# alexoz12v2/cuda-optix-pathtracing

Hardware: AMD Instinct MI355X
Metric: Msamples/s (paths x spp / s) (higher is better)
Workload: dtype f32

## Files before the change

### cuda-optix-pathtracing_amd/__init__.py

```python
from .binding import (
    DmtError,
    Renderer,
    bvh_validate,
    bvh_check,
    lbvh_reference,
    BVH_BUILD_HOST,
    BVH_BUILD_DEVICE,
    BVH_BUILT_BY_HOST,
    BVH_BUILT_BY_DEVICE,
    BVH_BUILT_BY_HOST_AFTER_DEVICE,
    bvh_refit_reference,
    BVH_UPDATE_REBUILD,
    BVH_UPDATE_REFIT,
    BVH_UPDATE_AUTO,
    BVH_UPDATED_NONE,
    BVH_UPDATED_REFIT,
    BVH_UPDATED_REBUILD,
    BVH_UPDATED_REBUILD_AFTER_REFIT,
    light_tree_pmfs,
    light_tree_ref_select,
    envmap_tables,
    texture_mip_chain,
    texture_footprint,
    temporal_defaults,
    camera_project,
    lens_rays,
    shutter_times,
    motion_positions,
    motion_bvh_validate,
    smooth_normals,
    opacity_eval,
    OPACITY_NONE,
    medium_segment,
    medium_values,
    phase_hg,
    medium_grid_march,
    medium_spectrum_event,
    mip_level_count,
    TEXFILTER_LEVEL0,
    TEXFILTER_REFERENCE,
    build_library,
    library_path,
    load_library,
)
from . import host_scene
from . import multigpu
```

### cuda-optix-pathtracing_amd/binding.py

```python
import ctypes as C
import subprocess
from pathlib import Path

import numpy as np

_HERE = Path(__file__).resolve().parent
_CSRC = _HERE / "csrc"
_LIB = None

DMT_ACCEL_BRUTE_FORCE = 0
DMT_ACCEL_BVH = 1
BVH_BUILD_HOST = 0
BVH_BUILD_DEVICE = 1
BVH_BUILT_BY_HOST = 0
BVH_BUILT_BY_DEVICE = 1
BVH_BUILT_BY_HOST_AFTER_DEVICE = 2
BVH_UPDATE_REBUILD = 0
BVH_UPDATE_REFIT = 1
BVH_UPDATE_AUTO = 2
BVH_UPDATED_NONE = 0
BVH_UPDATED_REFIT = 1
BVH_UPDATED_REBUILD = 2
BVH_UPDATED_REBUILD_AFTER_REFIT = 3

# ... 20 lines not shown
    global _LIB
    if _LIB is None:
        so = library_path()
        if not so.exists():
            raise DmtError(f"{so} is missing: run `python -c 'import __graft_entry__ as g; g.build()'` "
                           "(the HIP path has no fallback)")
        lib = C.CDLL(str(so))
        lib.dmt_last_error.restype = C.c_char_p
        lib.dmt_last_error.argtypes = [C.c_void_p]
        _LIB = lib
    return _LIB


EXPORTED_SYMBOLS = [
    "dmt_ctx_create", "dmt_ctx_destroy", "dmt_last_error", "dmt_upload_triangles", "dmt_upload_bsdfs",
    "dmt_upload_lights", "dmt_set_camera", "dmt_set_limits", "dmt_set_accel", "dmt_set_light_sampling", "dmt_light_tree_pmfs", "dmt_light_tree_ref_select", "dmt_set_bvh_strategy", "dmt_set_partition", "dmt_set_chunk", "dmt_render_profile",
    "dmt_upload_area_lights", "dmt_upload_textures", "dmt_upload_envmap", "dmt_clear_envmap", "dmt_envmap_tables", "dmt_test_envmap",
    "dmt_set_stream", "dmt_film_clear", "dmt_film_bind", "dmt_film_device_ptrs", "dmt_download_film",
    "dmt_render", "dmt_render_adaptive", "dmt_render_stats", "dmt_sync", "dmt_sched_diag", "dmt_kernel_time", "dmt_kernel_info", "dmt_bvh_validate", "dmt_brute_cull_plan", "dmt_brute_cull_box_plan", "dmt_brute_cull_box_records", "dmt_cull_box_test", "dmt_test_triangle_intersect",
    "dmt_test_sampler", "dmt_test_camera_rays", "dmt_test_bsdf", "dmt_test_bsdf_ng", "dmt_test_material", "dmt_test_light", "dmt_test_half",
    "dmt_test_trace_samples", "dmt_test_trace_log", "dmt_test_closest_hit",
    "dmt_set_texture_filter", "dmt_texture_mip_chain", "dmt_texture_footprint", "dmt_test_texture_filter",
    "dmt_render_aovs", "dmt_upload_aovs", "dmt_download_aovs", "dmt_denoise_defaults", "dmt_denoise",
    "dmt_set_accel_build", "dmt_accel_build_info", "dmt_accel_download", "dmt_lbvh_reference", "dmt_bvh_check",
    "dmt_update_vertices", "dmt_update_vertices_device", "dmt_set_accel_update", "dmt_accel_update_info", "dmt_bvh_refit_reference",
    "dmt_download_aov_surface", "dmt_upload_aov_surface", "dmt_camera_project", "dmt_test_camera_project", "dmt_temporal_defaults",
    "dmt_denoise_temporal", "dmt_temporal_reset", "dmt_temporal_info", "dmt_temporal_download",
    "dmt_set_sampler_table", "dmt_sampler_table_plan", "dmt_test_sampler_table",
    "dmt_set_lens", "dmt_lens_info", "dmt_lens_rays", "dmt_focus_distance_at", "dmt_test_lens_values",
    "dmt_set_motion", "dmt_clear_motion", "dmt_set_shutter", "dmt_motion_info", "dmt_shutter_times", "dmt_motion_positions",
    "dmt_motion_bvh_validate", "dmt_test_shutter_times", "dmt_test_closest_hit_at",
    "dmt_upload_vertex_normals", "dmt_clear_vertex_normals", "dmt_vertex_normals_info", "dmt_smooth_normals",
    "dmt_test_shading_normal", "dmt_test_shading_normal_mapped",
    "dmt_set_ggx_batch", "dmt_ggx_batch_diag", "dmt_tri_kind_bits",
    "dmt_upload_opacity", "dmt_clear_opacity", "dmt_opacity_info", "dmt_opacity_eval", "dmt_test_opacity", "dmt_test_closest_hit_opacity",
    "dmt_set_medium", "dmt_clear_medium", "dmt_medium_info", "dmt_medium_segment", "dmt_medium_values", "dmt_phase_hg", "dmt_test_medium",
    "dmt_set_medium_grid", "dmt_set_medium_grid_device", "dmt_clear_medium_grid", "dmt_medium_grid_info", "dmt_medium_grid_march", "dmt_test_medium_grid",
    "dmt_set_medium_spectrum", "dmt_clear_medium_spectrum", "dmt_medium_spectrum_info", "dmt_medium_spectrum_event", "dmt_test_medium_spectrum",
]

SAMPLER_TABLE_OFF = 0
SAMPLER_TABLE_AUTO = 1
SAMPLER_TABLE_FORCE = 2


class SamplerTablePlanRecord(C.Structure):
    _fields_ = [("use", C.c_uint32), ("period_width", C.c_uint32), ("period_height", C.c_uint32), ("entry_bytes", C.c_uint32),
                ("slices", C.c_uint32), ("reserved", C.c_uint32), ("slice_bytes", C.c_uint64)]


def sampler_table_plan(width, height, owned_pixels, spp, chunk_spp, budget_bytes=0, mode=SAMPLER_TABLE_AUTO):
    lib = load_library()
    rec = SamplerTablePlanRecord()
    args = [int(width), int(height), C.c_uint64(int(owned_pixels)), C.c_uint32(int(spp)), C.c_uint32(int(chunk_spp)),
            C.c_uint64(int(budget_bytes)), int(mode)]
    rc = lib.dmt_sampler_table_plan(*args, C.byref(rec), None, C.c_uint32(0))
    if rc != 0:
        raise DmtError(f"dmt_sampler_table_plan failed ({rc})")
    lens = (C.c_uint32 * max(int(rec.slices), 1))()
    rc = lib.dmt_sampler_table_plan(*args, C.byref(rec), lens, C.c_uint32(int(rec.slices)))
    if rc != 0:
        raise DmtError(f"dmt_sampler_table_plan failed ({rc})")
    out = {name: int(getattr(rec, name)) for name, _ in SamplerTablePlanRecord._fields_ if name != "reserved"}
    out["use"] = bool(rec.use)
    out["slice_spp"] = [int(x) for x in lens[:int(rec.slices)]]
    return out

# ... 56 lines not shown

def shutter_times(width, height, open, close, pxs, pys, ss):
    lib = load_library()
    pxs, pys, ss = _i32(pxs), _i32(pys), _i32(ss)
    n = pxs.shape[0]
    assert pys.shape[0] == n and ss.shape[0] == n
    t = np.zeros(n, np.float32)
    rc = lib.dmt_shutter_times(int(width), int(height), C.c_float(open), C.c_float(close), int(n), _p(pxs), _p(pys), _p(ss), _p(t))
    if rc != 0:
        raise DmtError(f"dmt_shutter_times failed ({rc})")
    return t


def motion_positions(xs0, ys0, zs0, xs1, ys1, zs1, t):
    lib = load_library()
    a = [_f32(v).reshape(-1) for v in (xs0, ys0, zs0, xs1, ys1, zs1)]
    n = a[0].size // 4
    assert all(v.size == 4 * n for v in a)
    out = [np.zeros(4 * n, np.float32) for _ in range(3)]
    rc = lib.dmt_motion_positions(*[_p(v) for v in a], C.c_size_t(n), C.c_float(t), *[_p(v) for v in out])
    if rc != 0:
        raise DmtError(f"dmt_motion_positions failed ({rc})")
    return tuple(out)


def motion_bvh_validate(xs0, ys0, zs0, xs1, ys1, zs1):
    lib = load_library()
    a = [_f32(v).reshape(-1) for v in (xs0, ys0, zs0, xs1, ys1, zs1)]
    n = a[0].size // 4
    assert all(v.size == 4 * n for v in a)
    nc, pc, d = C.c_int(), C.c_int(), C.c_int()
    rc = lib.dmt_motion_bvh_validate(*[_p(v) for v in a], C.c_size_t(n), C.byref(nc), C.byref(pc), C.byref(d))
    return {"ok": rc == 0, "node_count": nc.value, "pair_count": pc.value, "depth": d.value}


def smooth_normals(xs, ys, zs, crease_degrees=180.0):
    lib = load_library()
    xs, ys, zs = _f32(xs).reshape(-1), _f32(ys).reshape(-1), _f32(zs).reshape(-1)
    n = xs.size // 4
    assert xs.size == 4 * n and ys.size == 4 * n and zs.size == 4 * n
    out = np.zeros((n, 9), np.float32)
    rc = lib.dmt_smooth_normals(_p(xs), _p(ys), _p(zs), C.c_size_t(n), C.c_float(crease_degrees), _p(out))
    if rc != 0:
        raise DmtError(f"dmt_smooth_normals failed ({rc})")
    return out


def _u32(a):
    return np.ascontiguousarray(a, np.uint32).reshape(-1)


def medium_segment(box_min, box_max, o, d, t_hit):
    lib = load_library()
    o, d = _f32(o).reshape(-1, 3), _f32(d).reshape(-1, 3)
    t = _f32(t_hit).reshape(-1)
    n = o.shape[0]
    assert d.shape[0] == n and t.shape[0] == n
    seg, hit = np.zeros((n, 2), np.float32), np.zeros(n, np.int32)
    rc = lib.dmt_medium_segment(_p(_f32(box_min, (3,))), _p(_f32(box_max, (3,))), int(n), _p(o), _p(d), _p(t), _p(seg), _p(hit))
    if rc != 0:
        raise DmtError(f"dmt_medium_segment failed ({rc})")
    return seg, hit.astype(bool)


def medium_values(h, depth):
    lib = load_library()
# ... 636 lines not shown
        return nodes[:info["nodes"]].copy(), pairs[:info["pairs"]].copy()

    def set_light_sampling(self, mode):
        self._check(self._lib.dmt_set_light_sampling(self._ctx, int(mode)), "dmt_set_light_sampling")

    def set_texture_filter(self, mode):
        self._check(self._lib.dmt_set_texture_filter(self._ctx, int(mode)), "dmt_set_texture_filter")

    def set_bvh_strategy(self, strategy, paths_per_pass=0):
        self._check(self._lib.dmt_set_bvh_strategy(self._ctx, int(strategy), C.c_uint64(int(paths_per_pass))), "dmt_set_bvh_strategy")

    def set_partition(self, rank, world):
        self._check(self._lib.dmt_set_partition(self._ctx, int(rank), int(world)), "dmt_set_partition")

    def set_chunk(self, samples_per_item):
        self._check(self._lib.dmt_set_chunk(self._ctx, C.c_uint32(samples_per_item)), "dmt_set_chunk")

    def set_sampler_table(self, mode, budget_bytes=0):
        self._check(self._lib.dmt_set_sampler_table(self._ctx, int(mode), C.c_uint64(int(budget_bytes))), "dmt_set_sampler_table")

    def set_ggx_batch(self, batch):
        self._check(self._lib.dmt_set_ggx_batch(self._ctx, C.c_uint32(int(batch))), "dmt_set_ggx_batch")

    def ggx_batch(self):
        out = (C.c_uint64 * 5)()
        self._check(self._lib.dmt_ggx_batch_diag(self._ctx, out), "dmt_ggx_batch_diag")
        return int(out[4])

    def tri_kind_bits(self, triangles):
        out = np.zeros((int(triangles) + 31) // 32, np.uint32)
        self._check(self._lib.dmt_tri_kind_bits(self._ctx, out.ctypes.data_as(C.c_void_p), C.c_uint64(out.size)), "dmt_tri_kind_bits")
        return out

    def set_stream(self, stream_ptr):
        self._check(self._lib.dmt_set_stream(self._ctx, C.c_void_p(stream_ptr)), "dmt_set_stream")

    def film_clear(self):
        self._check(self._lib.dmt_film_clear(self._ctx), "dmt_film_clear")

    def film_bind(self, mean_ptr, m2_ptr):
        self._check(self._lib.dmt_film_bind(self._ctx, C.c_void_p(mean_ptr), C.c_void_p(m2_ptr)), "dmt_film_bind")

    def film_device_ptrs(self):
        a, b = C.c_void_p(), C.c_void_p()
        self._check(self._lib.dmt_film_device_ptrs(self._ctx, C.byref(a), C.byref(b)), "dmt_film_device_ptrs")
        return a.value, b.value

    def download_film(self):
        mean = np.zeros((self.height, self.width, 4), np.float32)
        m2 = np.zeros((self.height, self.width, 4), np.float32)
        self._check(self._lib.dmt_download_film(self._ctx, _p(mean), _p(m2)), "dmt_download_film")
        return mean, m2

    def render(self, spp, sample_offset=0, region=None):
        x0, y0, x1, y1 = region if region is not None else (0, 0, self.width, self.height)
        self._check(self._lib.dmt_render(self._ctx, C.c_uint32(sample_offset), C.c_uint32(spp), int(x0), int(y0),
                                         int(x1), int(y1)), "dmt_render")

    def render_adaptive(self, threshold, max_spp, step_spp, min_spp=0, region=None):
        x0, y0, x1, y1 = region if region is not None else (0, 0, self.width, self.height)
        rounds, samples = C.c_uint32(0), C.c_uint64(0)
        self._check(self._lib.dmt_render_adaptive(self._ctx, C.c_uint32(min_spp), C.c_uint32(max_spp), C.c_uint32(step_spp),
                                                  C.c_float(threshold), int(x0), int(y0), int(x1), int(y1), C.byref(rounds),
                                                  C.byref(samples)), "dmt_render_adaptive")
        return int(rounds.value), int(samples.value)

# ... 297 lines not shown
```

### cuda-optix-pathtracing_amd/csrc/dmt_hip.hip

```cpp
#include <hip/hip_runtime.h>

#include <algorithm>
#include <cassert>
#include <chrono>
#include <cmath>
#include <cstddef>
#include <cstdio>
#include <cstdlib>
#include <cstring>
#include <limits>
#include <map>
#include <memory>
#include <new>
#include <string>
#include <vector>

#include "../../include/dmt_hip.h"
#include "pt_device.hpp"
#include "medium.hpp"
#include "medium_grid.hpp"
#include "bvh_device.hpp"
#include "bvh_gpu_build.hpp"
#include "devbuf.hpp"
#include "envmap.hpp"
// ... 59 lines not shown
  float2 const* samTabLens;
  uint32_t samTabS0, samTabPw, samTabPh;
  float lensR, lensD;
  int maxDepth;
  int shadeThreshold;
  EnvView env;
  uint32_t const* areaOf;
  uint32_t const* areaTri;
  float const* areaLe;
  uint32_t areaCount;
  uint32_t const* texRgba;
  int32_t const* texDesc;
  uint32_t const* matTex;
  float const* triUv;
  LightTreeNode const* lightTree;
  LightTreeRefNode const* lightTreeRef;
  unsigned long long* stats;
  float texCfr[12];
  float texMinDx[3], texMinDy[3];
  float texSppScale;
  uint32_t const* texMip;
  int32_t const* texMipDesc;
  MotionView motion;
  VtxNormalRec const* vtxNormals;
  OpacityRec const* opacity;
  float opacityCutoff8;
  uint32_t ggxBatchT;
  float* ggxQueue;
  uint32_t const* triKindBits;
  uint32_t triKindInline[2];
  MediumParams medium;
  MediumGridParams mediumGrid;
  MediumSpectrumParams mediumSpectrum;
};

typedef RenderParams const DMT_CONST_AS* KArgs;
DMT_DEV KArgs kargs_base() { return (KArgs)__builtin_amdgcn_kernarg_segment_ptr(); }
DMT_DEV KArgs kargs(KArgs p) {
  asm volatile("" : "+s"(p));
  return p;
}
DMT_DEV SceneView load_scene(KArgs k) {
  k = kargs(k);
  SceneView s;
  s.tris = k->scene.tris, s.post = k->scene.post, s.bsdfs = k->scene.bsdfs, s.lights = k->scene.lights;
  s.infLights = k->scene.infLights, s.triCount = k->scene.triCount, s.bsdfCount = k->scene.bsdfCount;
  s.lightCount = k->scene.lightCount, s.infLightCount = k->scene.infLightCount;
  return s;
}
DMT_DEV BvhView load_bvh(KArgs k) {
  k = kargs(k);
  BvhView b;
  b.nodes = k->bvh.nodes, b.pairs = k->bvh.pairs, b.overflow = k->bvh.overflow, b.overflowStride = k->bvh.overflowStride;
  return b;
}

DMT_DEV EnvView load_env(KArgs k) {
  k = kargs(k);
  EnvView e;
  e.func = k->env.func, e.cdf = k->env.cdf, e.rowInt = k->env.rowInt, e.mFunc = k->env.mFunc, e.mCdf = k->env.mCdf;
  e.rgb = k->env.rgb, e.mInt = k->env.mInt, e.w = k->env.w, e.h = k->env.h;
  e.qx = k->env.qx, e.qy = k->env.qy, e.qz = k->env.qz, e.qw = k->env.qw;
  return e;
}

#ifndef DMT_SECTION_TIMING
// ... 119 lines not shown
  static_assert(!(F & kFeatVtxNormals) || !(F & ~(kFeatVtxNormals | kFeatBvh | kFeatEnv | kFeatTex)), "vertex normals: the plain, env-map and texture rows only");
  static_assert(!(F & kFeatMedium) || !(F & ~(kFeatMedium | kFeatMediumGrid | kFeatMediumSpectrum | kFeatBvh | kFeatEnv)), "medium: the plain and env-map rows only");
  static_assert(!(F & kFeatMediumGrid) || ((F & kFeatMedium) && !(F & ~(kFeatMediumGrid | kFeatMediumSpectrum | kFeatMedium | kFeatBvh | kFeatEnv))), "medium grid: with the medium, on the plain and env-map rows only");
  static_assert(!(F & kFeatMediumSpectrum) || ((F & kFeatMedium) && !(F & ~(kFeatMediumSpectrum | kFeatMediumGrid | kFeatMedium | kFeatBvh | kFeatEnv))), "medium spectrum: with the medium, on the plain and env-map rows only");
  SceneView const sc = load_scene(k);
  int const maxDepth = kargs(k)->maxDepth;
  if constexpr (F & kFeatMedium) {
    int const mv = medium_vertex<F>(k, st, sc, bestTri, bu, bv);
    if (mv != MV_THROUGH) return mv == MV_ENDED;
  }
  if constexpr (F & kFeatEnv) {
    if (bestTri < 0) {
      EnvView const env = load_env(k);
      float pdfLight = 0.f;
      f3 const Le = env_eval_dir(env, ray_dir(st), pdfLight);
      if (st.depth == 0 || st.lastSpecular)
        st.L = st.L + st.beta * Le;
      else
        st.L = st.L + st.beta * (st.lastPdf / (st.lastPdf + pdfLight)) * Le;
      return true;
    }
  }
  if (bestTri < 0) {
    if (sc.infLightCount > 0) {
      uint32_t const li = pick_index(st.rng.get1D(), sc.infLightCount);
      Rec32 const light = sc.infLights[li];
      float const pmf = 1.f / float(sc.infLightCount);
      if (light_type(light) == LT_ENV) st.L = st.L + st.beta * light_intensity(light) / pmf;
    }
    sect_mark(4);
    return true;
  }
  f3 const rd = ray_dir(st);
  Hit const hit = shade_hit<F>(k, sc, bestTri, bu, bv, rd);
  uint32_t nAll = sc.lightCount;
  if constexpr (F & kFeatArea) {
    KArgs const ka = kargs(k);
    nAll += ka->areaCount;
    uint32_t const ai = ka->areaOf[bestTri];
    if (ai != 0xFFFFFFFFu) {
      f3 const o = mk3(st.rp.ox.x, st.rp.oy.x, st.rp.oz.x);
      float const pl = area_pdf(sc.post[bestTri], rd, dot(hit.pos - o, rd));
      if (pl > 0.f) {
        f3 const Le = mk3(ka->areaLe[3 * ai], ka->areaLe[3 * ai + 1], ka->areaLe[3 * ai + 2]);
        if (st.depth == 0 || st.lastSpecular) {
          st.L = st.L + st.beta * Le;
        } else {
          float const a = st.lastPdf, b = pl * ((F & kFeatEnv) ? 0.5f : 1.f) / float(nAll);
          st.L = st.L + st.beta * Le * ((a * a) / (a * a + b * b));
        }
      }
    }
  }
  sect_mark(4);
  if (st.depth >= maxDepth) return true;

  f3 const wo = -rd;
  Rec32 rec = sc.bsdfs[hit.matId];
  f3 ns = hit.normal;
  if constexpr (F & kFeatVtxNormals) ns = shading_normal_at(k, bestTri, bu, bv, hit.normal);
  Rec32 rec2{};
  float mix = 0.f;
  bool blend = false;
  constexpr bool FILT = (F & kFeatTexFilter) != 0;
  TexDiff td{0.f, 0.f, 0.f, 0.f};
  if constexpr (FILT) {
    if (st.depth == 0) td = tex_footprint(k, bestTri, hit.pos, hit.normal);
  }
  if constexpr (F & kFeatBlend) {
    if (hi16(rec.w[1]) == BS_GGX_BLEND) {
      mix = blend_metallic<FILT>(k, rec, hit.matId, bestTri, bu, bv, td);
      rec.w[1] = (rec.w[1] & 0x0000FFFFu) | (uint32_t(BS_GGX_DIEL) << 16);
      rec2 = sc.bsdfs[hit.matId + 1u];
      if (mix >= 1.f) rec = rec2;
      else blend = mix > 0.f;
    }
  }
  if constexpr (F & (kFeatTex | kFeatBlend)) {
    if (!(F & kFeatBlend) || kargs(k)->matTex != nullptr) {
      ns = apply_material_textures<FILT>(k, rec, hit.matId, bestTri, bu, bv, ns, td);
      if (blend) (void)apply_material_textures<FILT>(k, rec2, hit.matId + 1u, bestTri, bu, bv, hit.normal, td);
    }
  }
#if DMT_SECTION_TIMING
  {
    bool const ggx = hi16(rec.w[1]) != BS_OREN;
    unsigned long long const all = __ballot(1), mg = __ballot(ggx);
    if (int(__ffsll((long long)all)) - 1 == int(threadIdx.x & 63u)) {
      unsigned long long* const acc = s_sectAcc[threadIdx.x >> 6];
      acc[11] += mg ? 1u : 0u, acc[12] += uint32_t(__popcll(mg)), acc[13] += 1u, acc[14] += uint32_t(__popcll(all));
    }
// ... 84 lines not shown
        f3 C;
        if (ls.delta) {
          C = st.beta * Le * f / pmf;
        } else {
          float const w = sqr(pmf * ls.pdf) / sqr(pmf * ls.pdf + bsdfPdf);
          C = Le * f * st.beta * w;
        }
        if (pending) {
          bool occ;
          if constexpr (F & kFeatBvh) {
            occ = bvh_any(load_bvh(k), true, pendO, pendD, pendMax, blockIdx.x * blockDim.x + threadIdx.x);
          } else {
            PathState tmp = st;
            set_shadow_ray(tmp, pendO, pendD);
            tmp.smax = pendMax;
            int bt;
            float tu, tvv;
            trace_pair_brute<false>(k, tmp, false, true, bt, tu, tvv, occ);
          }
          if (!occ) st.L = st.L + pendC;
        }
        pending = true, pendC = C, pendMax = ls.distance;
        pendO = offset_ray_origin(hit.pos, hit.error, hit.normal, ls.direction), pendD = ls.direction;
      }
      if (pending) {
        put_C(pendC);
        set_shadow_ray(st, pendO, pendD);
        st.smax = pendMax;
        st.hasShadow = true;
      }
    }
  }
  if (!envNee && !areaNee && !treeNee && sc.lightCount > 0) {
    uint32_t li = 0;
    float pmf = 0.f;
    bool picked = true;
    if constexpr (F & kFeatLightTree) {
      float treePmf = 0.f;
      int const sel = lt_select(kargs(k)->lightTree, hit.pos.x, hit.pos.y, hit.pos.z, hit.normal.x, hit.normal.y, hit.normal.z, uLight, treePmf);
      picked = sel >= 0;
      li = picked ? uint32_t(sel) : 0u;
      pmf = ((F & kFeatEnv) ? 0.5f : 1.f) * treePmf;
    } else {
      li = pick_index(uLight, (F & kFeatArea) ? nAll : sc.lightCount);
      pmf = ((F & kFeatEnv) ? 0.5f : 1.f) / float((F & kFeatArea) ? nAll : sc.lightCount);
    }
    Rec32 const light = sc.lights[li];
    LightSample const ls = sample_light(light, hit.pos, uLight2, st.lastT, hit.normal);
    sect_mark(6);
    if (picked && ls.valid()) {
      float bsdfPdf = 0.f;
      f3 const f = eval_material(ls.direction, bsdfPdf);
      if (!is_zero(f)) {
        f3 const Le = eval_light(light, ls);
        if (ls.delta) {
          put_C(st.beta * Le * f / pmf);
        } else {
          float const w = sqr(pmf * ls.pdf) / sqr(pmf * ls.pdf + bsdfPdf);
          put_C(Le * f * st.beta * w);
        }
        set_shadow_ray(st, offset_ray_origin(hit.pos, hit.error, hit.normal, ls.direction), ls.direction);
        st.smax = ls.distance;
        st.hasShadow = true;
      }
    }
  }

  if constexpr (F & kFeatMedium) {
    if (st.hasShadow) medium_attenuate_pending<F>(k, st);
  }
  sect_mark(7);
  f2 const u2 = st.rng.get2D();
  float const uc = st.rng.get1D();
  BsdfSample bs = sample_bsdf(b, wo, ns, hit.normal, u2, uc);
  if constexpr (F & kFeatBlend) {
    if (blend) {
      BsdfSample sC = sample_bsdf(b2, wo, ns, hit.normal, u2, uc);
      sC.f = bs.f * (1.f - mix) + sC.f * mix;
      sC.pdf = blend_pdf(bs.pdf, sC.pdf);
      sC.eta = 1.f;
      bs = sC;
    }
  }
  sect_mark(8);
  if (!bs.valid()) return true;
  st.lastT = bs.refract;
  if constexpr (F & (kFeatEnv | kFeatArea)) st.lastPdf = bs.pdf, st.lastSpecular = bs.delta;
  set_ray(st, offset_ray_origin(hit.pos, hit.error, hit.normal, bs.wi), bs.wi);
  st.beta = st.beta * (bs.f * fabsf(dot(bs.wi, hit.normal)) / bs.pdf);
  float const rrBeta = max3(st.beta * bs.eta);
  if (rrBeta < 1 && st.depth > 1) {
    float const q = fmaxf(0.f, 1.f - rrBeta);
    if (st.rng.get1D() < q) return true;
    st.beta = st.beta / (1 - q);
  }
  ++st.depth;
  sect_mark(9);
// ... 1358 lines not shown
  if (device_ordinal < 0 || device_ordinal >= count) {
    g_createError = "device ordinal out of range";
    return DMT_ERR_INVALID;
  }
  std::unique_ptr<dmt_ctx> ctx(new (std::nothrow) dmt_ctx());
  if (!ctx) return DMT_ERR_INVALID;
  ctx->device = device_ordinal;
  hipError_t e = hipSetDevice(device_ordinal);
  if (e == hipSuccess) e = hipStreamCreateWithFlags(&ctx->ownStream, hipStreamNonBlocking);
  hipDeviceProp_t prop{};
  if (e == hipSuccess) e = hipGetDeviceProperties(&prop, device_ordinal);
  if (e == hipSuccess) e = ctx->launch.allocate();
  int bpcBvh = 0;
  if (e == hipSuccess)
    e = hipOccupancyMaxActiveBlocksPerMultiprocessor(&bpcBvh, reinterpret_cast<void const*>(k_megakernel_bvh), 256, 0);
  if (e != hipSuccess) {
    g_createError = std::string("dmt_ctx_create: ") + hipGetErrorString(e);
    if (ctx->ownStream) (void)hipStreamDestroy(ctx->ownStream);
    return DMT_ERR_HIP;
  }
  ctx->stream = ctx->ownStream;
  ctx->launch.cuCount = prop.multiProcessorCount;
  ctx->ac.blocksPerCUBvh = bpcBvh > 0 ? bpcBvh : 1;
  ctx->launch.fromEnv();
  if (char const* e5 = std::getenv("DMT_BVH_SHADE_THRESHOLD")) {
    int const v = std::atoi(e5);
    ctx->ac.shadeThresholdEnv = v < 1 ? 0 : (v > 64 ? 64 : v);
  }
  if (char const* e6 = std::getenv("DMT_BRUTE_CULL")) {
    int const v = std::atoi(e6);
    ctx->bruteCull = v == 0 ? 0 : v == 1 ? 1 : 2;
  }
  if (char const* e7 = std::getenv("DMT_TRI_KIND_INLINE")) ctx->surf.kind.allowInline = std::atoi(e7) != 0;
  *out = ctx.release();
  return DMT_OK;
}

int dmt_ctx_destroy(dmt_ctx* ctx) {
  if (!ctx) return DMT_ERR_INVALID;
  (void)hipSetDevice(ctx->device);
  (void)hipStreamSynchronize(ctx->stream);
  for (auto& ev : ctx->launch.timing.events) {
    (void)hipEventDestroy(ev.first);
    (void)hipEventDestroy(ev.second);
  }
  if (ctx->ownStream) (void)hipStreamDestroy(ctx->ownStream);
  delete ctx;
  return DMT_OK;
}

const char* dmt_last_error(const dmt_ctx* ctx) { return ctx ? ctx->err.c_str() : g_createError.c_str(); }

int dmt_upload_triangles(dmt_ctx* ctx, const float* xs, const float* ys, const float* zs,
                         const uint32_t* mat_id, size_t count) {
  if (!ctx) return DMT_ERR_INVALID;
  if ((count && (!xs || !ys || !zs || !mat_id)) || count > 0x7FFFFFFFu)
    return fail(ctx, DMT_ERR_INVALID, "dmt_upload_triangles: null array or count out of range");
  HIP_TRY(ctx, hipSetDevice(ctx->device));
  std::vector<TriIsect> a;
  std::vector<TriPost> b;
  packSoup(xs, ys, zs, mat_id, count, a, b);
  uint32_t maxMat = 0;
  for (size_t i = 0; i < count; ++i)
    if (mat_id[i] > maxMat) maxMat = mat_id[i];
  DevBuf<TriIsect> tris;
  DevBuf<TriPost> post;
// ... 434 lines not shown
```

### cuda-optix-pathtracing_amd/csrc/surface_host.hpp

```cpp
#pragma once

namespace {

int buildMipChain(uint8_t const* rgba, int w, int h, std::vector<uint32_t>& out) {
  int levels = 0;
  for (int a = w, b = h; a > 0 || b > 0; a >>= 1, b >>= 1) ++levels;
  out.clear();
  std::vector<uint8_t> prev(rgba, rgba + 4 * size_t(w) * size_t(h)), cur;
  int pw = w, ph = h;
  for (int l = 1; l < levels; ++l) {
    int const cw = std::max(1, w >> l), ch = std::max(1, h >> l);
    cur.assign(4 * size_t(cw) * size_t(ch), 0);
    for (int v = 0; v < ch; ++v)
      for (int u = 0; u < cw; ++u) {
        bool const x1 = 2 * u + 1 < pw, y1 = 2 * v + 1 < ph;
        float const scale = (x1 && y1) ? 0.25f : (x1 || y1) ? 0.5f : 1.f;
        uint32_t word = 0;
        for (int c = 0; c < 4; ++c) {
          auto at = [&](int x, int y) { return float(prev[4 * (size_t(y) * size_t(pw) + size_t(x)) + size_t(c)]) / 255.f; };
          float sum = at(2 * u, 2 * v);
          if (x1) sum += at(2 * u + 1, 2 * v);
          if (y1) sum += at(2 * u, 2 * v + 1);
          if (x1 && y1) sum += at(2 * u + 1, 2 * v + 1);
          float const t = scale * sum * 255.f;
// ... 101 lines not shown
  HIP_TRY(ctx, hipSetDevice(ctx->device));
  HIP_TRY(ctx, hipStreamSynchronize(ctx->stream));
  SurfaceState::Emissive& area = ctx->surf.area = SurfaceState::Emissive{};
  if (count == 0 || !ctx->haveTris) return DMT_OK;
  std::vector<uint32_t> of(ctx->triCount, 0xFFFFFFFFu);
  for (uint32_t k = 0; k < count; ++k) {
    if (triangle_index[k] >= ctx->triCount) return fail(ctx, DMT_ERR_INVALID, "area light refers to a triangle outside the uploaded soup");
    of[triangle_index[k]] = k;
  }
  HIP_TRY(ctx, area.of.assign(of.data(), of.size()));
  HIP_TRY(ctx, area.tri.assign(triangle_index, count));
  HIP_TRY(ctx, area.le.assign(radiance_rgb, 3 * size_t(count)));
  area.count = count;
  return DMT_OK;
}

int dmt_tri_kind_bits(dmt_ctx* ctx, uint32_t* out, uint64_t words) {
  if (!ctx) return DMT_ERR_INVALID;
  SurfaceState::Kind const& kind = ctx->surf.kind;
  size_t const n = kind.words.size();
  if (words < n || (n && !out)) return fail(ctx, DMT_ERR_INVALID, "dmt_tri_kind_bits: room for (triangles + 31) / 32 words is needed");
  if (n == 0) return DMT_OK;
  if (kind.bits.get()) {
    HIP_TRY(ctx, hipSetDevice(ctx->device));
    HIP_TRY(ctx, hipMemcpy(out, kind.bits.get(), n * sizeof(uint32_t), hipMemcpyDeviceToHost));
  } else {
    RenderParams P{};
    ctx->surf.fill(P);
    for (size_t w = 0; w < n; ++w) out[w] = w < 2 ? P.triKindInline[w] : 0u;
  }
  return DMT_OK;
}

int dmt_upload_textures(dmt_ctx* ctx, const uint8_t* rgba8, uint64_t texel_count, const int32_t* desc3, uint32_t texture_count,
                        const uint32_t* mat_tex4, uint32_t bsdf_count, const float* tri_uv6, uint64_t triangle_count) {
  if (!ctx) return DMT_ERR_INVALID;
  HIP_TRY(ctx, hipSetDevice(ctx->device));
  HIP_TRY(ctx, hipStreamSynchronize(ctx->stream));
  ctx->surf.texturesReplaced();
  SurfaceState::Textures& tex = ctx->surf.tex;
  if (texture_count == 0) return DMT_OK;
  if (!rgba8 || !desc3 || !mat_tex4 || !tri_uv6 || texel_count == 0 || bsdf_count == 0 || triangle_count == 0)
    return fail(ctx, DMT_ERR_INVALID, "dmt_upload_textures: null array or zero count");
  if (!descriptorsInside(desc3, texture_count, texel_count, INT32_MAX))
    return fail(ctx, DMT_ERR_INVALID, "dmt_upload_textures: texture descriptor outside the texel array");
  for (uint32_t b = 0; b < bsdf_count; ++b)
    for (int j = 0; j < 3; ++j) {
      uint32_t const t = mat_tex4[4 * size_t(b) + size_t(j)];
      if (t != 0xFFFFFFFFu && t >= texture_count) return fail(ctx, DMT_ERR_INVALID, "dmt_upload_textures: material refers to a texture that does not exist");
    }
  std::vector<uint32_t> mip;
  std::vector<int32_t> mipDesc(2 * size_t(texture_count));
  for (uint32_t k = 0; k < texture_count; ++k) {
    std::vector<uint32_t> chain;
    mipDesc[2 * k] = buildMipChain(rgba8 + 4 * size_t(desc3[3 * k]), desc3[3 * k + 1], desc3[3 * k + 2], chain);
    if (mip.size() + chain.size() > size_t(INT32_MAX)) return fail(ctx, DMT_ERR_INVALID, "dmt_upload_textures: MIP chains too large");
    mipDesc[2 * k + 1] = int32_t(mip.size());
    mip.insert(mip.end(), chain.begin(), chain.end());
  }
  HIP_TRY(ctx, tex.mip.assign(mip.data(), mip.size()));
  HIP_TRY(ctx, tex.mipDesc.assign(mipDesc.data(), mipDesc.size()));
  HIP_TRY(ctx, tex.rgba.assign(rgba8, size_t(texel_count)));
  HIP_TRY(ctx, tex.desc.assign(desc3, 3 * size_t(texture_count)));
  HIP_TRY(ctx, tex.matTex.assign(mat_tex4, 4 * size_t(bsdf_count)));
  HIP_TRY(ctx, tex.triUv.assign(tri_uv6, 6 * size_t(triangle_count)));
  tex.count = texture_count, tex.matTexCount = bsdf_count, tex.triUvCount = size_t(triangle_count);
// ... 134 lines not shown
```

### cuda-optix-pathtracing_amd/csrc/surface_state.hpp

```cpp
#pragma once

namespace {

struct SurfaceState {
  struct Textures {
    DevBuf<uint32_t> rgba;
    DevBuf<int32_t> desc;
    DevBuf<uint32_t> matTex;
    DevBuf<float> triUv;
    DevBuf<uint32_t> mip;
    DevBuf<int32_t> mipDesc;
    uint32_t count = 0, matTexCount = 0;
    size_t triUvCount = 0;
  } tex;
  int texFilter = DMT_TEXFILTER_LEVEL0;
  float texFoot[19] = {};
  struct VertexNormals {
    DevBuf<VtxNormalRec> recs;
    bool have = false;
    uint64_t smooth = 0;
  } vn;
  struct Opacity {
    DevBuf<OpacityRec> recs;
    bool have = false;
    float cutoff = 0.f;
    uint64_t cutoutTris = 0;
    uint32_t cutoutMats = 0;
  } op;
  struct Emissive {
    DevBuf<uint32_t> of, tri;
    DevBuf<float> le;
    uint32_t count = 0;
  } area;
  struct Kind {
    std::vector<uint8_t> matGgx;
    std::vector<uint32_t> words;
    DevBuf<uint32_t> bits;
    bool allowInline = true;
  } kind;
  static constexpr size_t kTriKindInlineTris = 64;

  hipError_t soupReplaced(std::vector<uint32_t> const& matId) {
    vn = VertexNormals{}, op = Opacity{}, area = Emissive{};
    return buildKind(matId);
  }
  hipError_t bsdfsReplaced(void const* bsdf32, uint32_t count, std::vector<uint32_t> const& matId) {
    op = Opacity{};
    kind.matGgx.assign(count, 0);
    for (uint32_t i = 0; i < count; ++i) {
      uint32_t w1;
      memcpy(&w1, static_cast<unsigned char const*>(bsdf32) + 32 * size_t(i) + 4, 4);
      kind.matGgx[i] = (w1 >> 16) == BS_GGX_DIEL || (w1 >> 16) == BS_GGX_COND;
    }
    return buildKind(matId);
  }
  void texturesReplaced() { tex = Textures{}, op = Opacity{}; }

  hipError_t buildKind(std::vector<uint32_t> const& matId) {
    kind.words.assign((matId.size() + 31) / 32, 0u);
    for (size_t i = 0; i < matId.size(); ++i)
      if (matId[i] < kind.matGgx.size() && kind.matGgx[matId[i]]) kind.words[i >> 5] |= 1u << (i & 31);
    DevBuf<uint32_t> fresh;
    if (!kind.allowInline || matId.size() > kTriKindInlineTris) {
      hipError_t const e = fresh.assign(kind.words.data(), kind.words.size());
      if (e != hipSuccess) {
        kind.words.assign(kind.words.size(), 0u), kind.bits.reset();
        return e;
      }
    }
    kind.bits = std::move(fresh);
    return hipSuccess;
  }

  bool texturesMatch(uint32_t bsdfCount, size_t triCount) const { return tex.count == 0 || (tex.matTexCount == bsdfCount && tex.triUvCount == triCount); }

  void fill(RenderParams& P) const {
    P.areaOf = area.of.get(), P.areaTri = area.tri.get(), P.areaLe = area.le.get(), P.areaCount = area.count;
    P.triKindBits = kind.bits.get();
    for (size_t w = 0; !P.triKindBits && w < 2 && w < kind.words.size(); ++w) P.triKindInline[w] = kind.words[w];
    if (vn.have) P.vtxNormals = vn.recs.get();
    if (op.have) P.opacity = op.recs.get(), P.opacityCutoff8 = op.cutoff * 255.f;
    if (tex.count > 0) {
      P.texRgba = tex.rgba.get(), P.texDesc = tex.desc.get(), P.matTex = tex.matTex.get(), P.triUv = tex.triUv.get();
      P.texMip = tex.mip.get(), P.texMipDesc = tex.mipDesc.get();
      memcpy(P.texCfr, texFoot, 12 * sizeof(float));
      memcpy(P.texMinDx, texFoot + 12, 3 * sizeof(float));
      memcpy(P.texMinDy, texFoot + 15, 3 * sizeof(float));
      P.texSppScale = texFoot[18];
    }
  }
};

}
```

### include/dmt_hip.h

```cpp
#ifndef DMT_HIP_H
#define DMT_HIP_H

#include <stddef.h>
#include <stdint.h>

#ifdef __cplusplus
extern "C" {
#endif

typedef struct dmt_ctx dmt_ctx;

typedef struct dmt_camera {
  float dir[3];
  float pos[3];
  int32_t width;
  int32_t height;
  int32_t spp;
  float focal_length;
  float sensor_size;
} dmt_camera;

enum {
  DMT_OK = 0,
  DMT_ERR_INVALID = 1,
// ... 98 lines not shown
#define DMT_SAMPLER_TABLE_OFF 0
#define DMT_SAMPLER_TABLE_AUTO 1
#define DMT_SAMPLER_TABLE_FORCE 2
int dmt_set_sampler_table(dmt_ctx* ctx, int mode, uint64_t budget_bytes);
typedef struct dmt_sampler_table_plan_record {
  uint32_t use;
  uint32_t period_width, period_height;
  uint32_t entry_bytes;
  uint32_t slices;
  uint32_t reserved;
  uint64_t slice_bytes;
} dmt_sampler_table_plan_record;
int dmt_sampler_table_plan(int width, int height, uint64_t owned_pixels, uint32_t spp, uint32_t chunk_spp, uint64_t budget_bytes,
                           int mode, dmt_sampler_table_plan_record* out, uint32_t* slice_spp, uint32_t slice_cap);
int dmt_set_stream(dmt_ctx* ctx, void* hip_stream);

int dmt_film_clear(dmt_ctx* ctx);
int dmt_film_bind(dmt_ctx* ctx, void* d_mean, void* d_m2);
int dmt_film_device_ptrs(dmt_ctx* ctx, void** d_mean, void** d_m2);
int dmt_download_film(dmt_ctx* ctx, float* mean4, float* m24);

int dmt_render(dmt_ctx* ctx, uint32_t sample_offset, uint32_t spp, int x0, int y0, int x1, int y1);
int dmt_render_adaptive(dmt_ctx* ctx, uint32_t min_spp, uint32_t max_spp, uint32_t step_spp, float threshold,
                        int x0, int y0, int x1, int y1, uint32_t* rounds, uint64_t* samples);
int dmt_render_stats(dmt_ctx* ctx, uint32_t sample_offset, uint32_t spp, int x0, int y0, int x1, int y1,
                     uint64_t* stats6);
int dmt_render_profile(dmt_ctx* ctx, uint32_t sample_offset, uint32_t spp, int x0, int y0, int x1, int y1,
                       uint64_t* stats16);
int dmt_sync(dmt_ctx* ctx);
int dmt_sched_diag(dmt_ctx* ctx, uint64_t* out8, int reset);
int dmt_set_ggx_batch(dmt_ctx* ctx, uint32_t batch);
int dmt_ggx_batch_diag(dmt_ctx* ctx, uint64_t* out5);
int dmt_tri_kind_bits(dmt_ctx* ctx, uint32_t* out, uint64_t words);
int dmt_kernel_time(dmt_ctx* ctx, double* total_ms, uint64_t* launches, int reset);
int dmt_kernel_info(dmt_ctx* ctx, int* vgprs, int* sgprs, int* lds_bytes, int* blocks_per_cu,
                    int* cu_count);

int dmt_bvh_validate(const float* xs, const float* ys, const float* zs, size_t count, int* node_count,
                     int* depth, int* max_leaf);

enum {
  DMT_BVH_BUILD_HOST = 0,
  DMT_BVH_BUILD_DEVICE = 1,
};
enum {
  DMT_BVH_BUILT_BY_HOST = 0,
  DMT_BVH_BUILT_BY_DEVICE = 1,
  DMT_BVH_BUILT_BY_HOST_AFTER_DEVICE = 2,
};
int dmt_set_accel_build(dmt_ctx* ctx, int mode);
typedef struct dmt_accel_build_record {
  int32_t builder;
  int32_t depth;
  uint32_t triangles;
  uint32_t nodes;
  uint32_t pairs;
  uint32_t reserved;
  double build_ms;
  uint64_t temp_bytes;
} dmt_accel_build_record;
int dmt_accel_build_info(dmt_ctx* ctx, dmt_accel_build_record* out);
int dmt_accel_download(dmt_ctx* ctx, void* nodes64, size_t node_cap, uint32_t* pair_orig2, size_t pair_cap);
int dmt_lbvh_reference(const float* xs, const float* ys, const float* zs, size_t count, int max_depth, void* nodes64,
                       size_t node_cap, uint32_t* pair_orig2, size_t pair_cap, uint32_t* node_count, uint32_t* pair_count,
                       int* depth, int* abandoned);
int dmt_bvh_check(const void* nodes64, size_t node_count, const uint32_t* pair_orig2, size_t pair_count, const float* xs,
// ... 127 lines not shown
```

Before: 6321.

## Prefetch per-triangle BSDF records and specialise single-light NEE

Builds a per-triangle table of 32-byte BSDF records for scenes with at most 32768 triangles. The shading kernel fetches the record by triangle index before shade_hit, so the load no longer waits on the material-id lookup and can overlap with shading. A separate path for the no-feature variant with exactly one light reads that light through the constant address space and skips index selection. Costs are extra device memory per triangle, extra registers held across shade_hit, and more code in the kernel.

```diff
diff --git a/cuda-optix-pathtracing_amd/__init__.py b/cuda-optix-pathtracing_amd/__init__.py
--- a/cuda-optix-pathtracing_amd/__init__.py
+++ b/cuda-optix-pathtracing_amd/__init__.py
@@ -29,6 +29,7 @@
     motion_positions,
     motion_bvh_validate,
     smooth_normals,
+    tri_bsdf_build,
     opacity_eval,
     OPACITY_NONE,
     medium_segment,
diff --git a/cuda-optix-pathtracing_amd/binding.py b/cuda-optix-pathtracing_amd/binding.py
--- a/cuda-optix-pathtracing_amd/binding.py
+++ b/cuda-optix-pathtracing_amd/binding.py
@@ -76,7 +76,7 @@
     "dmt_motion_bvh_validate", "dmt_test_shutter_times", "dmt_test_closest_hit_at",
     "dmt_upload_vertex_normals", "dmt_clear_vertex_normals", "dmt_vertex_normals_info", "dmt_smooth_normals",
     "dmt_test_shading_normal", "dmt_test_shading_normal_mapped",
-    "dmt_set_ggx_batch", "dmt_ggx_batch_diag", "dmt_tri_kind_bits",
+    "dmt_set_ggx_batch", "dmt_ggx_batch_diag", "dmt_tri_kind_bits", "dmt_tri_bsdf_records", "dmt_tri_bsdf_build",
     "dmt_upload_opacity", "dmt_clear_opacity", "dmt_opacity_info", "dmt_opacity_eval", "dmt_test_opacity", "dmt_test_closest_hit_opacity",
     "dmt_set_medium", "dmt_clear_medium", "dmt_medium_info", "dmt_medium_segment", "dmt_medium_values", "dmt_phase_hg", "dmt_test_medium",
     "dmt_set_medium_grid", "dmt_set_medium_grid_device", "dmt_clear_medium_grid", "dmt_medium_grid_info", "dmt_medium_grid_march", "dmt_test_medium_grid",
@@ -199,6 +199,18 @@
     nc, pc, d = C.c_int(), C.c_int(), C.c_int()
     rc = lib.dmt_motion_bvh_validate(*[_p(v) for v in a], C.c_size_t(n), C.byref(nc), C.byref(pc), C.byref(d))
     return {"ok": rc == 0, "node_count": nc.value, "pair_count": pc.value, "depth": d.value}
+
+
+def tri_bsdf_build(bsdfs, mat_id):
+    lib = load_library()
+    lib.dmt_tri_bsdf_build.restype = C.c_int64
+    b = np.ascontiguousarray(bsdfs, np.uint8).reshape(-1, 32)
+    m = np.ascontiguousarray(mat_id, np.uint32).reshape(-1)
+    out = np.zeros((m.size, 32), np.uint8)
+    n = lib.dmt_tri_bsdf_build(_p(b), C.c_uint32(b.shape[0]), _p(m), C.c_uint64(m.size), _p(out), C.c_uint64(m.size))
+    if n < 0:
+        raise DmtError(f"dmt_tri_bsdf_build failed ({-n})")
+    return out[:n]
 
 
 def smooth_normals(xs, ys, zs, crease_degrees=180.0):
@@ -901,6 +913,14 @@
         self._check(self._lib.dmt_tri_kind_bits(self._ctx, out.ctypes.data_as(C.c_void_p), C.c_uint64(out.size)), "dmt_tri_kind_bits")
         return out
 
+    def tri_bsdf_records(self, triangles):
+        out = np.zeros((max(int(triangles), 1), 32), np.uint8)
+        self._lib.dmt_tri_bsdf_records.restype = C.c_int64
+        n = self._lib.dmt_tri_bsdf_records(self._ctx, out.ctypes.data_as(C.c_void_p), C.c_uint64(int(triangles)))
+        if n < 0:
+            self._check(int(-n), "dmt_tri_bsdf_records")
+        return out[:n]
+
     def set_stream(self, stream_ptr):
         self._check(self._lib.dmt_set_stream(self._ctx, C.c_void_p(stream_ptr)), "dmt_set_stream")
 
diff --git a/cuda-optix-pathtracing_amd/csrc/dmt_hip.hip b/cuda-optix-pathtracing_amd/csrc/dmt_hip.hip
--- a/cuda-optix-pathtracing_amd/csrc/dmt_hip.hip
+++ b/cuda-optix-pathtracing_amd/csrc/dmt_hip.hip
@@ -115,6 +115,7 @@
   MediumParams medium;
   MediumGridParams mediumGrid;
   MediumSpectrumParams mediumSpectrum;
+  Rec32 const* triBsdf;
 };
 
 typedef RenderParams const DMT_CONST_AS* KArgs;
@@ -300,6 +301,13 @@
     return true;
   }
   f3 const rd = ray_dir(st);
+  constexpr bool kTriBsdfRow = F != kFeatTex && F != (kFeatEnv | kFeatBlend);
+  Rec32 const* triBsdf = nullptr;
+  Rec32 recTri{};
+  if constexpr (kTriBsdfRow) {
+    triBsdf = kargs(k)->triBsdf;
+    if (triBsdf != nullptr) recTri = triBsdf[bestTri];
+  }
   Hit const hit = shade_hit<F>(k, sc, bestTri, bu, bv, rd);
   uint32_t nAll = sc.lightCount;
   if constexpr (F & kFeatArea) {
@@ -324,7 +332,10 @@
   if (st.depth >= maxDepth) return true;
 
   f3 const wo = -rd;
-  Rec32 rec = sc.bsdfs[hit.matId];
+  Rec32 rec = kTriBsdfRow ? recTri : sc.bsdfs[hit.matId];
+  if constexpr (kTriBsdfRow) {
+    if (triBsdf == nullptr) rec = sc.bsdfs[hit.matId];
+  }
   f3 ns = hit.normal;
   if constexpr (F & kFeatVtxNormals) ns = shading_normal_at(k, bestTri, bu, bv, hit.normal);
   Rec32 rec2{};
@@ -475,37 +486,49 @@
     }
   }
   if (!envNee && !areaNee && !treeNee && sc.lightCount > 0) {
-    uint32_t li = 0;
-    float pmf = 0.f;
-    bool picked = true;
-    if constexpr (F & kFeatLightTree) {
-      float treePmf = 0.f;
-      int const sel = lt_select(kargs(k)->lightTree, hit.pos.x, hit.pos.y, hit.pos.z, hit.normal.x, hit.normal.y, hit.normal.z, uLight, treePmf);
-      picked = sel >= 0;
-      li = picked ? uint32_t(sel) : 0u;
-      pmf = ((F & kFeatEnv) ? 0.5f : 1.f) * treePmf;
+    auto nee = [&](Rec32 const& light, float pmf, bool picked) __attribute__((always_inline)) {
+      LightSample const ls = sample_light(light, hit.pos, uLight2, st.lastT, hit.normal);
+      sect_mark(6);
+      if (picked && ls.valid()) {
+        float bsdfPdf = 0.f;
+        f3 const f = eval_material(ls.direction, bsdfPdf);
+        if (!is_zero(f)) {
+          f3 const Le = eval_light(light, ls);
+          if (ls.delta) {
+            put_C(st.beta * Le * f / pmf);
+          } else {
+            float const w = sqr(pmf * ls.pdf) / sqr(pmf * ls.pdf + bsdfPdf);
+            put_C(Le * f * st.beta * w);
+          }
+          set_shadow_ray(st, offset_ray_origin(hit.pos, hit.error, hit.normal, ls.direction), ls.direction);
+          st.smax = ls.distance;
+          st.hasShadow = true;
+        }
+      }
+    };
+    constexpr bool kOneLightRow = F == 0;
+    if (kOneLightRow && sc.lightCount == 1u) {
+      auto const* const only = to_const_as(sc.lights);
+      Rec32 light;
+#pragma unroll
+      for (int w = 0; w < 8; ++w) light.w[w] = only[0].w[w];
+      nee(light, ((F & kFeatEnv) ? 0.5f : 1.f) / float(sc.lightCount), true);
     } else {
-      li = pick_index(uLight, (F & kFeatArea) ? nAll : sc.lightCount);
-      pmf = ((F & kFeatEnv) ? 0.5f : 1.f) / float((F & kFeatArea) ? nAll : sc.lightCount);
-    }
-    Rec32 const light = sc.lights[li];
-    LightSample const ls = sample_light(light, hit.pos, uLight2, st.lastT, hit.normal);
-    sect_mark(6);
-    if (picked && ls.valid()) {
-      float bsdfPdf = 0.f;
-      f3 const f = eval_material(ls.direction, bsdfPdf);
-      if (!is_zero(f)) {
-        f3 const Le = eval_light(light, ls);
-        if (ls.delta) {
-          put_C(st.beta * Le * f / pmf);
-        } else {
-          float const w = sqr(pmf * ls.pdf) / sqr(pmf * ls.pdf + bsdfPdf);
-          put_C(Le * f * st.beta * w);
-        }
-        set_shadow_ray(st, offset_ray_origin(hit.pos, hit.error, hit.normal, ls.direction), ls.direction);
-        st.smax = ls.distance;
-        st.hasShadow = true;
+      uint32_t li = 0;
+      float pmf = 0.f;
+      bool picked = true;
+      if constexpr (F & kFeatLightTree) {
+        float treePmf = 0.f;
+        int const sel = lt_select(kargs(k)->lightTree, hit.pos.x, hit.pos.y, hit.pos.z, hit.normal.x, hit.normal.y, hit.normal.z, uLight, treePmf);
+        picked = sel >= 0;
+        li = picked ? uint32_t(sel) : 0u;
+        pmf = ((F & kFeatEnv) ? 0.5f : 1.f) * treePmf;
+      } else {
+        li = pick_index(uLight, (F & kFeatArea) ? nAll : sc.lightCount);
+        pmf = ((F & kFeatEnv) ? 0.5f : 1.f) / float((F & kFeatArea) ? nAll : sc.lightCount);
       }
+      Rec32 const light = sc.lights[li];
+      nee(light, pmf, picked);
     }
   }
 
@@ -1930,6 +1953,7 @@
     ctx->bruteCull = v == 0 ? 0 : v == 1 ? 1 : 2;
   }
   if (char const* e7 = std::getenv("DMT_TRI_KIND_INLINE")) ctx->surf.kind.allowInline = std::atoi(e7) != 0;
+  if (char const* e8 = std::getenv("DMT_TRI_BSDF")) ctx->surf.triBsdf.enabled = std::atoi(e8) != 0;
   *out = ctx.release();
   return DMT_OK;
 }
diff --git a/cuda-optix-pathtracing_amd/csrc/surface_host.hpp b/cuda-optix-pathtracing_amd/csrc/surface_host.hpp
--- a/cuda-optix-pathtracing_amd/csrc/surface_host.hpp
+++ b/cuda-optix-pathtracing_amd/csrc/surface_host.hpp
@@ -157,6 +157,30 @@
   return DMT_OK;
 }
 
+int64_t dmt_tri_bsdf_records(dmt_ctx* ctx, void* out32, uint64_t cap) {
+  if (!ctx) return -int64_t(DMT_ERR_INVALID);
+  SurfaceState::TriBsdf const& tb = ctx->surf.triBsdf;
+  if (tb.count == 0) return 0;
+  if (cap < tb.count || !out32) return -int64_t(fail(ctx, DMT_ERR_INVALID, "dmt_tri_bsdf_records: room for one 32-byte record per triangle is needed"));
+  auto copy = [&]() -> int {
+    HIP_TRY(ctx, hipSetDevice(ctx->device));
+    HIP_TRY(ctx, hipMemcpy(out32, tb.recs.get(), tb.count * sizeof(Rec32), hipMemcpyDeviceToHost));
+    return DMT_OK;
+  };
+  int const rc = copy();
+  return rc == DMT_OK ? int64_t(tb.count) : -int64_t(rc);
+}
+
+int64_t dmt_tri_bsdf_build(const void* bsdf32, uint32_t bsdf_count, const uint32_t* mat_id, uint64_t triangle_count, void* out32, uint64_t cap) {
+  if ((bsdf_count && !bsdf32) || (triangle_count && !mat_id)) return -int64_t(DMT_ERR_INVALID);
+  std::vector<Rec32> mats(bsdf_count), recs;
+  if (bsdf_count) memcpy(mats.data(), bsdf32, 32 * size_t(bsdf_count));
+  if (!SurfaceState::makeTriBsdf(mats.data(), mats.size(), mat_id, size_t(triangle_count), recs)) return 0;
+  if (cap < recs.size() || !out32) return -int64_t(DMT_ERR_INVALID);
+  memcpy(out32, recs.data(), recs.size() * sizeof(Rec32));
+  return int64_t(recs.size());
+}
+
 int dmt_upload_textures(dmt_ctx* ctx, const uint8_t* rgba8, uint64_t texel_count, const int32_t* desc3, uint32_t texture_count,
                         const uint32_t* mat_tex4, uint32_t bsdf_count, const float* tri_uv6, uint64_t triangle_count) {
   if (!ctx) return DMT_ERR_INVALID;
diff --git a/cuda-optix-pathtracing_amd/csrc/surface_state.hpp b/cuda-optix-pathtracing_amd/csrc/surface_state.hpp
--- a/cuda-optix-pathtracing_amd/csrc/surface_state.hpp
+++ b/cuda-optix-pathtracing_amd/csrc/surface_state.hpp
@@ -39,10 +39,18 @@
     bool allowInline = true;
   } kind;
   static constexpr size_t kTriKindInlineTris = 64;
+  struct TriBsdf {
+    std::vector<Rec32> mats;
+    DevBuf<Rec32> recs;
+    size_t count = 0;
+    bool enabled = true;
+  } triBsdf;
+  static constexpr size_t kTriBsdfMaxTris = 32768;
 
   hipError_t soupReplaced(std::vector<uint32_t> const& matId) {
     vn = VertexNormals{}, op = Opacity{}, area = Emissive{};
-    return buildKind(matId);
+    hipError_t const e = buildKind(matId), e2 = buildTriBsdf(matId);
+    return e != hipSuccess ? e : e2;
   }
   hipError_t bsdfsReplaced(void const* bsdf32, uint32_t count, std::vector<uint32_t> const& matId) {
     op = Opacity{};
@@ -52,7 +60,10 @@
       memcpy(&w1, static_cast<unsigned char const*>(bsdf32) + 32 * size_t(i) + 4, 4);
       kind.matGgx[i] = (w1 >> 16) == BS_GGX_DIEL || (w1 >> 16) == BS_GGX_COND;
     }
-    return buildKind(matId);
+    triBsdf.mats.resize(count);
+    if (count) memcpy(triBsdf.mats.data(), bsdf32, 32 * size_t(count));
+    hipError_t const e = buildKind(matId), e2 = buildTriBsdf(matId);
+    return e != hipSuccess ? e : e2;
   }
   void texturesReplaced() { tex = Textures{}, op = Opacity{}; }
 
@@ -72,12 +83,32 @@
     return hipSuccess;
   }
 
+  static bool makeTriBsdf(Rec32 const* mats, size_t matCount, uint32_t const* matId, size_t triCount, std::vector<Rec32>& out) {
+    out.clear();
+    if (triCount == 0 || triCount > kTriBsdfMaxTris) return false;
+    out.assign(triCount, Rec32{});
+    for (size_t i = 0; i < triCount; ++i)
+      if (matId[i] < matCount) out[i] = mats[matId[i]];
+    return true;
+  }
+  hipError_t buildTriBsdf(std::vector<uint32_t> const& matId) {
+    DevBuf<Rec32> fresh;
+    std::vector<Rec32> host;
+    hipError_t e = hipSuccess;
+    if (triBsdf.enabled && makeTriBsdf(triBsdf.mats.data(), triBsdf.mats.size(), matId.data(), matId.size(), host))
+      e = fresh.assign(host.data(), host.size());
+    if (e != hipSuccess) fresh.reset(), host.clear();
+    triBsdf.recs = std::move(fresh), triBsdf.count = host.size();
+    return e;
+  }
+
   bool texturesMatch(uint32_t bsdfCount, size_t triCount) const { return tex.count == 0 || (tex.matTexCount == bsdfCount && tex.triUvCount == triCount); }
 
   void fill(RenderParams& P) const {
     P.areaOf = area.of.get(), P.areaTri = area.tri.get(), P.areaLe = area.le.get(), P.areaCount = area.count;
     P.triKindBits = kind.bits.get();
     for (size_t w = 0; !P.triKindBits && w < 2 && w < kind.words.size(); ++w) P.triKindInline[w] = kind.words[w];
+    P.triBsdf = triBsdf.count ? triBsdf.recs.get() : nullptr;
     if (vn.have) P.vtxNormals = vn.recs.get();
     if (op.have) P.opacity = op.recs.get(), P.opacityCutoff8 = op.cutoff * 255.f;
     if (tex.count > 0) {
diff --git a/include/dmt_hip.h b/include/dmt_hip.h
--- a/include/dmt_hip.h
+++ b/include/dmt_hip.h
@@ -154,6 +154,8 @@
 int dmt_set_ggx_batch(dmt_ctx* ctx, uint32_t batch);
 int dmt_ggx_batch_diag(dmt_ctx* ctx, uint64_t* out5);
 int dmt_tri_kind_bits(dmt_ctx* ctx, uint32_t* out, uint64_t words);
+int64_t dmt_tri_bsdf_records(dmt_ctx* ctx, void* out, uint64_t cap);
+int64_t dmt_tri_bsdf_build(const void* bsdf32, uint32_t bsdf_count, const uint32_t* mat_id, uint64_t triangle_count, void* out, uint64_t cap);
 int dmt_kernel_time(dmt_ctx* ctx, double* total_ms, uint64_t* launches, int reset);
 int dmt_kernel_info(dmt_ctx* ctx, int* vgprs, int* sgprs, int* lds_bytes, int* blocks_per_cu,
                     int* cu_count);
```

Result: no change. 6375, median of 6 (+0.9%).
